# marella/ctransformers

Measured on NVIDIA H100. Metric: decode tokens/s Llama-2-7B Q4_K_M b=1, higher is better.
Workload: dtype int8 (q4_K/q6_K weights x q8_K activations, mma.sync u8 x s8 -> exact int32), fp32 combine in the reference's order

## Files before the change

### ctransformers_b200/csrc/engine.cu

```cuda
#include "engine.cuh"

#include <algorithm>
#include <chrono>
#include <cstdio>
#include <cstring>
#include <stdexcept>

#include "attention.cuh"
#include "grammar.hpp"
#include "grammar_gpu.cuh"
#include "matvec.cuh"
#include "prefill.cuh"
#include "repack.cuh"
#include "sample_gpu.cuh"
#include "score_gpu.cuh"
#include "stream.cuh"
#include "tables.hpp"
#include "tp_nccl.hpp"

namespace ctb {

#define CTB_CUDA(expr)                                                                                         \
  do {                                                                                                         \
    cudaError_t e__ = (expr);                                                                                  \
// ... 328 lines not shown
  xa_ = (float*)alloc(hp_.n_embd * 4); xb_ = (float*)alloc(hp_.n_embd * 4);
  qkv_ = (float*)alloc(qkv * 4);
  attn_ = (float*)alloc(hp_.n_embd * 4); attn_o_ = (float*)alloc(hp_.n_embd * 4);
  ffn_ = (float*)alloc((size_t)nff_ * 4);
  ffn2_ = (float*)alloc((size_t)nff_ * 4);
  d_logits_ = (float*)alloc((size_t)hp_.n_vocab * 4);
  d_embd_ = (float*)alloc(hp_.n_embd * 4);
  {
    const size_t nl = (size_t)hp_.n_seq * hp_.n_vocab, ne = (size_t)hp_.n_seq * hp_.n_embd, bytes = (nl + ne) * 4 + (size_t)hp_.n_seq * 8;
    kept_logits_ = (float*)alloc(bytes);
    kept_embd_ = kept_logits_ + nl;
    kept_pick_ = (int*)(kept_embd_ + ne);
    CTB_CUDA(cudaMemset(kept_logits_, 0, bytes));
  }
  d_sync_ = (unsigned*)alloc(64);
  CTB_CUDA(cudaMemset(d_state_, 0, 64));
  CTB_CUDA(cudaMemset(d_sync_, 0, 64));
  h_logits_ = HostMem((size_t)hp_.n_vocab * 4);
  h_embd_ = HostMem((size_t)hp_.n_embd * 4);
  memset(h_logits_.get(), 0, (size_t)hp_.n_vocab * 4);
  memset(h_embd_.get(), 0, (size_t)hp_.n_embd * 4);
  step_ring_ = StateRing(d_state_, 4, 512);

  if (const char* e = getenv("CTB_NO_PDL")) pdl_ = !(e[0] == '1');
  if (const char* e = getenv("CTB_NO_SPEC")) spec_on_ = !(e[0] == '1');
  if (const char* e = getenv("CTB_STEP_FUSE")) fused_ = !(e[0] == '0');
  if (const char* e = getenv("CTB_NO_PREFILL")) prefill_on_ = !(e[0] == '1');
  if (const char* e = getenv("CTB_PREFILL_MIN")) prefill_min_ = std::max(1, atoi(e));
  h_spec_tok_ = HostMem(16);
  {
// ... 239 lines not shown
    push_matvec(p, MVK_OUT);
    mark_exchange(first_op);

  }
  {
    StepOp op{};
    op.ph.kind = PH_PICK;
    op.ph.pk.logits = d_logits_; op.ph.pk.state = d_state_; op.ph.pk.out_tokens = nullptr; op.ph.pk.n = hp_.n_vocab;
    ops_.push_back(op);
  }
  bool any_stream = false;
  for (const StepOp& op : ops_) any_stream |= op.ph.kind == PH_MATVEC && op.stream;
  std::vector<Phase> phs;
  for (const StepOp& op : ops_) if (op.ph.kind != PH_XCHG && (op.ph.kind != PH_MATVEC || op.stream)) phs.push_back(op.ph);
  const StepLaunch sl = step_launch_plan(phs.data(), (int)phs.size(), sm_count_);
  step_grid_ = sl.grid; step_slots_ = sl.n_slots; step_smem_ = sl.smem; step_q3_ = sl.q3;
  if (const char* e = getenv("CTB_ST_SLOTS")) {
    const int want = atoi(e);
    if (want >= ST_W && want < step_slots_ && want % ST_W == 0) { step_smem_ -= (size_t)(step_slots_ - want) * ST_SLOT; step_slots_ = want; }
  }
  ring_attn_ = st_attn_ring_ok(hp_.n_ctx, step_slots_) && !getenv("CTB_NO_RING_ATTN");
  for (StepOp& op : ops_) if (op.ph.kind == PH_ATTN) op.ph.q6 = ring_attn_ ? 1 : 0;
  if (any_stream && step_slots_ < ST_W) throw std::runtime_error("model rows are too long for the step kernel's shared memory");
  if (any_stream) {
    CTB_CUDA(step_set_smem_limit(step_smem_));
    StepLaunch pl = sl;
    pl.n_slots = step_slots_; pl.smem = step_smem_;
    step_pair_ = step_pair_choose(pl, phs.data(), (int)phs.size());
  } else {
    fused_ = false;
  }
  d_prog_ = (Phase*)alloc((ops_.size() + 1) * sizeof(Phase), 256);
  d_prog_mv_ = (Phase*)alloc((ops_.size() + 1) * sizeof(Phase), 256);
  d_bounds_ = (int*)alloc((ops_.size() + 1) * (size_t)(sm_count_ + 1) * 4, 256);
  d_bounds_mv_ = (int*)alloc((ops_.size() + 1) * (size_t)(sm_count_ + 1) * 4, 256);
}

void Engine::upload_prog(Phase* dst, int* dst_bounds, const std::vector<StepOp>& ops) {
  std::vector<Phase> phs(ops.size());
  for (size_t i = 0; i < ops.size(); i++) phs[i] = ops[i].ph;
  CTB_CUDA(cudaMemcpy(dst, phs.data(), phs.size() * sizeof(Phase), cudaMemcpyHostToDevice));
  std::vector<Phase> run = phs;
  for (size_t i = 0; i < ops.size(); i++) if (ops[i].ph.kind == PH_XCHG || (ops[i].ph.kind == PH_MATVEC && !ops[i].stream)) run[i].kind = -1;
  const std::vector<int> b = step_bounds(run.data(), (int)run.size(), sm_count_);
  CTB_CUDA(cudaMemcpy(dst_bounds, b.data(), b.size() * 4, cudaMemcpyHostToDevice));
}

struct ProfMark {
  Event ev;
  int kind;
};

long Engine::enqueue_ops(const std::vector<StepOp>& ops, const Phase* d_prog, const int* d_bounds, int n, cudaStream_t st, bool fused,
                         std::vector<ProfMark>* marks) {
  long launches = 0;
  auto mark = [&](int kind) {
    if (!marks) return;
    marks->push_back({Event(cudaEventDefault), kind});
    CTB_CUDA(cudaEventRecord(marks->back().ev, st));
  };
  StepLaunch step_shape_;
  step_shape_.grid = step_grid_; step_shape_.n_slots = step_slots_; step_shape_.smem = step_smem_; step_shape_.gen = !attn_fast_hd(hp_.head_dim());
  step_shape_.q3 = step_q3_;
  step_shape_.pair = step_pair_;
  auto capable = [&](const StepOp& op) { return op.ph.kind != PH_XCHG && (op.ph.kind != PH_MATVEC || op.stream); };
  int i = 0;
  while (i < n) {
    const StepOp& op = ops[i];
    if (fused && capable(op)) {
      int j = i;
      while (j < n && capable(ops[j])) j++;
      mark(-1);
      CTB_CUDA(launch_step(step_shape_, st, d_prog + i, d_bounds + (size_t)i * (sm_count_ + 1), j - i, d_sync_, false, nullptr, tp_peer_));
      launches++;
      mark(0);
      i = j;
      continue;
    }
    mark(-1);
    switch (op.ph.kind) {
      case PH_EMBED:
        k_embed<<<1, 256, 0, st>>>(op.ph.em);
        launches++;
        mark(3);
        break;
      case PH_ATTN:
        CTB_CUDA(launch_kernel(attn_kernel(hp_.head_dim()), dim3(nh_, 1, attn_groups(hp_.head_dim())), dim3(ATTN_THREADS), attn_smem_bytes(hp_.n_ctx, hp_.head_dim()), st, pdl_, op.ph.at));
        launches++;
        mark(1);
        break;
      case PH_XCHG:
        tp_all_reduce(op.ph.em.out, op.ph.em.K, st);
        mark(3);
        break;
      case PH_PICK:
        k_argmax<<<1, ARGMAX_THREADS, 0, st>>>(d_logits_, hp_.n_vocab, d_state_ + 4);
        k_advance<<<1, 1, 0, st>>>(d_state_, d_tokens_out_.as<int>());
        launches += 2;
        mark(3);
        break;
      default:
        if (op.stream) {
          CTB_CUDA(launch_step(step_shape_, st, d_prog + i, d_bounds + (size_t)i * (sm_count_ + 1), 1, d_sync_));
        } else {
          const MVLaunch L = matvec_launch_shape(op.ph.mv, sm_count_);
          CTB_CUDA(launch_matvec_kernel(L, st, op.ph.mv, pdl_));
        }
        launches++;
        mark(0);
    }
    i++;
  }
  CTB_CUDA(cudaGetLastError());
  return launches;
}

int Engine::profile_step(int token, int n_past, double ms_by_kind[4], int count_by_kind[4]) {
  DeviceGuard dev_guard(device_);
// ... 45 lines not shown
  return (double)ms / reps;
}

long Engine::trace_step(int token, int n_past, unsigned long long* out, long cap_words) {
  DeviceGuard dev_guard(device_);
  if (tp_.world > 1) throw std::runtime_error("not available in tensor-parallel mode (every rank must run the same launches)");
  drop_lookahead();
  const int n = n_body_ + 1;
  for (int i = 0; i < n; i++)
    if (ops_[i].ph.kind == PH_MATVEC && !ops_[i].stream) return 0;
  const long need = 2L * n + 8L * n * step_grid_;
  if (need > cap_words) return -need;
  const DevMem buf((size_t)n * step_grid_ * 64);
  CTB_CUDA(cudaMemset(buf.get(), 0, (size_t)n * step_grid_ * 64));
  StepLaunch L;
  L.grid = step_grid_; L.n_slots = step_slots_; L.smem = step_smem_; L.gen = !attn_fast_hd(hp_.head_dim()); L.q3 = step_q3_; L.pair = step_pair_;
  for (int rep = 0; rep < 3; rep++) {
    put_step(token, n_past, n_past + 1);
    CTB_CUDA(launch_step(L, stream_, d_prog_, d_bounds_, n, d_sync_, false, buf.as<unsigned long long>()));
    CTB_CUDA(cudaStreamSynchronize(stream_));
  }
  for (int i = 0; i < n; i++) { out[2 * i] = (unsigned long long)ops_[i].ph.kind; out[2 * i + 1] = (unsigned long long)ops_[i].mvk; }
  CTB_CUDA(cudaMemcpy(out + 2 * n, buf.get(), (size_t)n * step_grid_ * 64, cudaMemcpyDeviceToHost));
  return n;
}

void Engine::build_graphs() {
  tokens_out_cap_ = std::max(hp_.n_ctx, 4096);
  d_tokens_out_ = DevMem((size_t)tokens_out_cap_ * 4);
  h_tokens_out_ = HostMem((size_t)tokens_out_cap_ * 4);
  const Stream cap(cudaStreamNonBlocking);
  ops_.back().ph.pk.out_tokens = d_tokens_out_.as<int>();
  upload_prog(d_prog_, d_bounds_, ops_);
  long launches = 0;
// ... 770 lines not shown
```

### ctransformers_b200/csrc/engine.cuh

```cuda
#pragma once
#include <cmath>
#include <memory>
#include <string>
#include <vector>

#include "cuda_owned.cuh"
#include "device_types.cuh"
#include "gguf.hpp"

namespace ctb {

struct TPShard {
  int rank = 0, world = 1;
  int head0 = 0, head1 = 0, kv0 = 0, kv1 = 0, ff0 = 0, ff1 = 0;
  void* comm = nullptr;
};
TPShard tp_shard(int n_embd, int n_head, int n_head_kv, int n_ff, int rank, int world);

struct HParams {
  bool falcon = false;
  int n_vocab = 0, n_ctx_train = 0, n_embd = 0, n_ff = 0, n_head = 0, n_head_kv = 0, n_layer = 0, n_rot = 0;
  float eps = 1e-5f, rope_base = 10000.f, rope_scale = 1.f;
  int n_ctx = 512;
  int n_seq = 1;
// ... 128 lines not shown
  int kv_high_ = 0;
  HostMem h_spec_tok_;
  HostMem h_dbg_;
  void after_eval(int next_pos);
  int sm_count_ = 132;

  void init(const GGUFFile& g);
  DevMat upload_matrix(const GGUFTensor& t, struct Uploader& up, int want_K, int want_M, int row0 = 0, int row1 = -1, int k0 = 0, int k1 = -1);
  const float* upload_vector(const GGUFFile& g, const std::string& name, bool required, int want_n);
  std::vector<StepOp> ops_;
  int n_body_ = 0;
  Phase* d_prog_ = nullptr;
  Phase* d_prog_mv_ = nullptr;
  int *d_bounds_ = nullptr, *d_bounds_mv_ = nullptr;
  unsigned* d_sync_ = nullptr;
  int step_grid_ = 0, step_slots_ = 0;
  size_t step_smem_ = 0;
  bool fused_ = true;
  bool step_q3_ = false;
  bool step_pair_ = false;
  bool ring_attn_ = false;
  void build_ops();
  void push_matvec(struct MVParams& p, int kind);
  void upload_prog(Phase* dst, int* dst_bounds, const std::vector<StepOp>& ops);
  long enqueue_ops(const std::vector<StepOp>& ops, const Phase* d_prog, const int* d_bounds, int n, cudaStream_t st, bool fused,
                   std::vector<ProfMark>* marks = nullptr);
  void build_graphs();
  bool eager_ = false;
  bool host_fresh_ = true;
  void host_views();
  DevMem d_sample_;
  HostMem h_sample_;
  void sample_enqueue(const SampleRow* rows, int R, bool picks);
  bool pieces_ready_ = false;
  DevMem d_pieces_, d_gm_, d_gm_rows_;
// ... 45 lines not shown
```

### ctransformers_b200/csrc/matvec.cuh

```cuda
#pragma once
#include "device_types.cuh"
#include "attention.cuh"

namespace ctb {

#ifndef CTB_THREADS
#define CTB_THREADS 512
#endif
constexpr int MV_THREADS = CTB_THREADS;
constexpr int MV_WARPS = MV_THREADS / 32;
constexpr int MV_ROWS = 4;
constexpr int MV_MAX_SEG = 3;

enum : int { NORM_NONE = 0, NORM_RMS = 1, NORM_LAYER = 2 };
enum : int { EPI_STORE = 0, EPI_ADD = 1, EPI_GELU = 2, EPI_ADD2 = 3, EPI_SILU = 4 };

#ifndef ST_WATCHDOG_NS
#define ST_WATCHDOG_NS 4000000000ull
#endif
#ifndef XC_WATCHDOG_NS
#define XC_WATCHDOG_NS 30000000000ull
#endif
enum WaitCode : int {
  W_GRID_BARRIER = 1, W_FOLD_FLAG, W_FREE_WEIGHT_SLOT, W_WEIGHT_ITEM, W_FREE_K_SLOT, W_FREE_V_SLOT, W_K_ITEM, W_V_ITEM, W_XCHG,
  W_PF_GRID_BARRIER, W_PF_FREE_SLOT, W_PF_WEIGHT_ITEM, W_PAIR, W_CODES
};
constexpr const char* WAIT_TEXT[] = {"?", "grid barrier (aux = phase)", "fold hand-off flag (aux = chunk)", "producer: free weight slot (aux = item)",
                                     "consumer: weight item (aux = item)", "producer: free K slot (attention)", "producer: free V slot (attention)",
                                     "consumer: K item (attention)", "consumer: V item (attention)", "tensor-parallel exchange: a peer's element (aux = exchange number)",
// ... 16 lines not shown
}

struct MVSeg {
  DevMat w;
  float* out;
  const float* res;
  const float* res2;
  int epi;
};

struct MVParams {
  const float* x;
  const float* x2;
  int x_mode;
  int x_parts, x_stride;
  float* sum_out;
  const float* norm_w;
  const float* norm_b;
  float* norm_out;
  float eps;
  int norm_mode;
  int K;
  int act;
  int nseg;
  MVSeg seg[MV_MAX_SEG];
  const uint16_t* silu_tab;
  const uint16_t* gelu_tab;
};

struct ActView {
// ... 209 lines not shown
    for (int l = 0; l < 32; l++)
#pragma unroll
      for (int i = 0; i < 16; i++) {
        float t = __shfl_sync(0xffffffffu, v[i], l);
        if (kind == NORM_TERM_DEV) t = __fsub_rn(t, mean);
        if (base + l * 16 + i < K) seq += kind == NORM_TERM_X ? (double)t : (double)__fmul_rn(t, t);
      }
  }
  return seq;
}

template <int NT, int BAR, bool XC, bool PAIR = false>
__device__ __forceinline__ float norm_stat(double s, double a, double g, bool a_is_s, int kind, float mean, const MVParams& xs, double* red,
                                           unsigned epoch, PairX* px = nullptr) {
  const int K = xs.K;
  if constexpr (PAIR) pair_sum2_max_f64<NT, BAR>(s, a, g, a_is_s, *px);
  else if (a_is_s) a = s = block_sum_f64<NT, BAR>(s, red);
  else block_sum2_max_f64<NT, BAR>(s, a, g, red);
  if (!isfinite(s) || (!a_is_s && __dmul_ru(a, g) < 0x1p52)) return (float)(s / (double)K);
  const double e = __dmul_ru(a, (double)K * 0x1.0000001p-52);
  const float lo = (float)(__dsub_rd(s, e) / (double)K), hi = (float)(__dadd_ru(s, e) / (double)K);
  if (lo == hi) return lo;
  const double seq = threadIdx.x < 32 ? seq_sum_warp0<XC>(xs.x, xs.x2, xs.x_mode, xs.x_parts, xs.x_stride, K, kind, mean, epoch) : 0.0;
  bar_sync<BAR, NT>();
  if (threadIdx.x == 0) red[0] = seq;
  bar_sync<BAR, NT>();
  return (float)(red[0] / (double)K);
}

__device__ __forceinline__ void norm_apply16(float (&v)[16], const float (&w)[16], const float (&bb)[16], int norm_mode, float mean, float scale, bool has_w,
                                             bool has_b) {
// ... 178 lines not shown
      }
    } else if (act == ACT_F16) {
      uint16_t* h = (uint16_t*)smem;
#pragma unroll
      for (int e = 0; e < 16; e++) if (e < valid) h[base + e] = f2h(v[e]);
    } else {
      float* f = (float*)smem;
#pragma unroll
      for (int e = 0; e < 16; e++) if (e < valid) f[base + e] = v[e];
    }
  }
  bar_sync<BAR, NT>();
}

template <int NT, int BAR>
__device__ __forceinline__ void stage_q8k_pair(const MVParams& xs, const NormPre& np, uint8_t* smem, double* red, PairX& px, bool write_norm) {
  const int K = xs.K, nb = K >> 8, norm_mode = xs.norm_mode, t = threadIdx.x, lane = t & 31;
  const int lo = pair_block0(nb, (int)px.rank) * 256, hi = pair_block0(nb, (int)px.rank + 1) * 256;
  const int base[2] = {lo + t * 16, lo + (t + NT) * 16};
  float v[2][16];
  load16x(xs, base[0], hi - base[0], v[0]);
  load16x(xs, base[1], hi - base[1], v[1]);
  float mean = 0.f, scale = 1.f;
  if (norm_mode == NORM_RMS) {
    double ss = 0.0;
#pragma unroll
    for (int h = 0; h < 2; h++)
#pragma unroll
      for (int e = 0; e < 16; e++) ss += (double)__fmul_rn(v[h][e], v[h][e]);
    const float m = norm_stat<NT, BAR, false, true>(ss, ss, 0.0, true, NORM_TERM_SQ, 0.f, xs, red, 0, &px);
    scale = __fdiv_rn(1.0f, __fsqrt_rn(__fadd_rn(m, xs.eps)));
  } else if (norm_mode == NORM_LAYER) {
    double s1 = 0.0, a1 = 0.0;
    unsigned emin = 255;
#pragma unroll
    for (int h = 0; h < 2; h++)
#pragma unroll
      for (int e = 0; e < 16; e++) {
        s1 += (double)v[h][e];
        a1 += (double)fabsf(v[h][e]);
// ... 233 lines not shown
```

### ctransformers_b200/csrc/stream.cuh

```cuda
#pragma once
#include <stdexcept>
#include <string>
#include "matvec.cuh"

namespace ctb {

#ifndef CTB_ST_WARPS
#define CTB_ST_WARPS 10
#endif
constexpr int ST_W = CTB_ST_WARPS;
constexpr int ST_NT = ST_W * 32;
constexpr int ST_THREADS = ST_NT + 32;
constexpr int ST_SLOT = 9216;
#ifndef CTB_ST_DEPTH
#define CTB_ST_DEPTH 2
#endif
constexpr int ST_MAX_DEPTH = CTB_ST_DEPTH;
constexpr int ST_MAX_SLOTS = ST_W * ST_MAX_DEPTH;
constexpr int ST_MAXT = 16;
constexpr int ST_ROWS = 16;
constexpr int ST_BAR = 1;
constexpr int ST_STATE = 6;

#ifndef CTB_CHUNK_Q3
// ... 365 lines not shown
    const uint32_t w0 = __vsub4((a0 & 0x0f0f0f0fu) | ((a2 & 0x03030303u) << 4), 0x20202020u);
    const uint32_t w1 = __vsub4((a1 & 0x0f0f0f0fu) | (((a2 >> 2) & 0x03030303u) << 4), 0x20202020u);
    const uint32_t w2 = __vsub4(((a0 >> 4) & 0x0f0f0f0fu) | (((a2 >> 4) & 0x03030303u) << 4), 0x20202020u);
    const uint32_t w3 = __vsub4(((a1 >> 4) & 0x0f0f0f0fu) | (((a2 >> 6) & 0x03030303u) << 4), 0x20202020u);
    const uint32_t sel = par ? 0x7531u : 0x6420u;
    const uint32_t S0 = __byte_perm(w0, w1, sel), S1 = __byte_perm(w2, w3, sel);
#pragma unroll
    for (int c = 0; c < 2; c++) {
      const int i = rr * 2 + c;
      r.p[i] = (float)scale_fold8(D[0][i], D[1][i], D[2][i], D[3][i], D[4][i], D[5][i], D[6][i], D[7][i], S0, S1);
    }
    r.dd[rr] = __fmul_rn(yd, h2f(rr ? d1 : d0));
  }
}

template <int TYPE, bool XC>
__device__ __forceinline__ void run_item(const uint8_t* slot, uint64_t* empty_bar, int nblk, int b0, int kc, bool last, const StAct& a, int lane,
                                         volatile float* mail, volatile int* flag, const MVSeg& sg, const MVParams& p, int row0) {
  constexpr int KB = StTraits<TYPE>::KB, BB = StTraits<TYPE>::BB, NM = StTraits<TYPE>::NM;
  Terms tr[KB];
  if (nblk == KB) {
#pragma unroll
    for (int i = 0; i < KB; i++) block_terms<TYPE>(slot + i * BB, b0 + i, a, lane, tr[i]);
  } else {
#pragma unroll
    for (int i = 0; i < KB; i++) {
      if (i < nblk) block_terms<TYPE>(slot + i * BB, b0 + i, a, lane, tr[i]);
      else { Terms z{}; tr[i] = z; }
    }
  }
  __syncwarp();
  if (lane == 0) mbar_arrive(empty_bar);

// ... 35 lines not shown
    u0 = __fadd_rn(u0, __shfl_xor_sync(0xffffffffu, u0, 2));
    u1 = __fadd_rn(u1, __shfl_xor_sync(0xffffffffu, u1, 2));
    u0 = __fadd_rn(u0, __shfl_xor_sync(0xffffffffu, u0, 1));
    u1 = __fadd_rn(u1, __shfl_xor_sync(0xffffffffu, u1, 1));
    float v = __fadd_rn(u0, u1);
    if (TYPE == GT_Q4_K) {
      float m = accm[rr];
      m = __fadd_rn(m, __shfl_xor_sync(0xffffffffu, m, 2));
      m = __fadd_rn(m, __shfl_xor_sync(0xffffffffu, m, 1));
      v = __fadd_rn(v, m);
    } else if (TYPE == GT_Q5_K) {
      v = __fadd_rn(v, __shfl_sync(0xffffffffu, accm[0], (lane & ~3) + rr));
    }
    out[rr] = v;
  }
  if (t < 2) {
    const int row = row0 + g + 8 * t;
    if (row < sg.w.M) {
      if (XC && a.xc) {
        const float v = epilogue(sg.epi, t ? out[1] : out[0], sg.res + row, sg.res2 + row, p);
        const XchgParams& xc = *a.xc;
        const size_t at = ((size_t)(a.epoch & 1u) * xc.world + xc.rank) * xc.n + row;
        for (int r = 0; r < xc.world; r++)
          asm volatile("st.volatile.global.v2.u32 [%0], {%1, %2};" ::"l"(xc.ll[r] + at), "r"(__float_as_uint(v)), "r"(a.epoch) : "memory");
      } else {
        store_epilogue(sg, p, row, t ? out[1] : out[0]);
      }
    }
  }
}

struct TileSpace {
  int tiles[MV_MAX_SEG], cost[MV_MAX_SEG], nseg, ntiles;
  long total;
  template <bool Q3 = true>
  __host__ __device__ __forceinline__ void init(const MVParams& p) {
    nseg = p.nseg; ntiles = 0; total = 0;
#pragma unroll
    for (int s = 0; s < MV_MAX_SEG; s++) {
      tiles[s] = s < p.nseg ? (p.seg[s].w.M + ST_ROWS - 1) / ST_ROWS : 0;
      cost[s] = s < p.nseg ? st_tile_cost<Q3>(p.seg[s].w.type) : 1;
      ntiles += tiles[s]; total += (long)tiles[s] * cost[s];
    }
// ... 34 lines not shown
  int q6;
  MVParams mv;
  AttnParams at;
  EmbedParams em;
  PickParams pk;
  XchgParams xc;
};

struct StepArgs {
  const Phase* prog;
  int n_phases;
  int n_slots;
  unsigned* sync;
  const int* bounds;
  unsigned long long* trace;
};

__device__ __forceinline__ unsigned ld_relaxed_u32(const unsigned* p) {
  unsigned v;
  asm volatile("ld.relaxed.gpu.global.u32 %0, [%1];" : "=r"(v) : "l"(p) : "memory");
  return v;
}
__device__ __forceinline__ unsigned ld_acquire_u32(const unsigned* p) {
  unsigned v;
  asm volatile("ld.acquire.gpu.global.u32 %0, [%1];" : "=r"(v) : "l"(p) : "memory");
  return v;
}

struct TileInfo { int seg, til, nch, type; };
template <bool Q3>
// ... 121 lines not shown
  const int n_cg = GEN ? attn_groups(ph.at.hd) : ph.at.hd / ATTN_CH, n_tasks = ph.at.n_head * n_cg, G = (int)gridDim.x;
  if (ph.q6) {
    const AttnRing ag = attn_ring_geom<GEN>(ph.at);
    for (int task = blockIdx.x; task < n_tasks; task += G) {
      if (task != (int)blockIdx.x) bar_sync<ST_BAR, ST_NT>();
      if (ag.T > 0) st_attn_task<GEN>(ph.at, act_smem, ring, full_bar, empty_bar, (uint32_t)(n_slots / ST_W), seq, ag, task / n_cg, task % n_cg, pick_v, red);
      seq += (uint32_t)(ag.n_k + attn_ring_nv<GEN>(ag, ph.at.hd, task % n_cg));
    }
  } else {
    for (int task = blockIdx.x; task < n_tasks; task += G) {
      if (task != (int)blockIdx.x) bar_sync<ST_BAR, ST_NT>();
      attn_body<ST_NT, ST_BAR, false, GEN>(ph.at, act_smem, task / n_cg, 0, task % n_cg, ph.at.state);
    }
  }
}
template <bool Q3, bool PAIR>
static __device__ __noinline__ uint32_t st_attn_phase_gen(const Phase& ph, uint8_t* act_smem, uint8_t* ring, uint64_t* full_bar, uint64_t* empty_bar, int n_slots,
                                                   uint32_t seq, float* pick_v, double* red) {
  st_attn_phase<true>(ph, act_smem, ring, full_bar, empty_bar, n_slots, seq, pick_v, red);
  return seq;
}

template <bool XC, bool GEN, bool Q3>
__device__ __forceinline__ void st_producer(const StepArgs& args, uint8_t* ring, uint64_t* full_bar, uint64_t* empty_bar) {
  const int lane = threadIdx.x & 31;
  const uint32_t S = (uint32_t)(args.n_slots / ST_W);
  const uint64_t weight_pol = l2_policy_evict_first();
  uint32_t seq = 0;
  for (int ip = 0; ip < args.n_phases; ip++) {
    const Phase* ph = args.prog + ip;
    if (ph->kind == PH_ATTN) {
// ... 23 lines not shown
            const RingPos rp = st_ring(n, S);
            const StItem it = st_item<Q3>(p, ti.seg, ti.type, ti.til, kc, nb);
            mbar_wait(&empty_bar[rp.slot], rp.parity ^ 1u, W_FREE_WEIGHT_SLOT, (int)n);
            mbar_expect_tx(&full_bar[rp.slot], it.bytes);
            bulk_g2s_hint(ring + (size_t)rp.slot * ST_SLOT, it.src, it.bytes, &full_bar[rp.slot], weight_pol);
          }
          __syncwarp();
        }
        __syncwarp();
        seq += (uint32_t)__popc(mask);
      }
    }
  }
}

template <bool XC, bool Q3, bool PAIR>
__device__ __forceinline__ void st_matvec_phase(const Phase& ph, const NormPre& np, uint8_t* ring, uint8_t* act_smem, double* red, uint64_t* full_bar, uint64_t* empty_bar,
                                                float (*mailbox)[ST_STATE * 32], int* flags, uint32_t S, uint32_t& seq, const int* tb, unsigned long long* tr,
                                                unsigned xc_base, PairX& px) {
  const MVParams& p = ph.mv;
  const int warp = threadIdx.x >> 5, lane = threadIdx.x & 31;
  const unsigned epoch = XC ? xc_base + (unsigned)ph.xc.index + 1u : 0u;
  if constexpr (PAIR) stage_q8k_pair<ST_NT, ST_BAR>(p, np, act_smem, red, px, blockIdx.x < 2);
  else stage_activation<ST_NT, ST_BAR, XC>(p, np, ACT_Q8_K, act_smem, red, blockIdx.x == 0, epoch);
  StAct a = st_act_extras<ST_NT, ST_BAR>(act_smem, p.K, ph.q6 != 0);
  a.xc = XC && ph.xc.role == 2 ? &ph.xc : nullptr;
  a.epoch = epoch;
  if (tr && threadIdx.x == 0) tr[1] = globaltimer_ns();
  bool first_item = tr != nullptr && threadIdx.x == 0;
  TileSpace ts;
  ts.init<Q3>(p);
  const int nb = p.K >> 8;
  const int T0 = tb[0], T1 = tb[1];
#pragma unroll 1
  for (int w0 = T0; w0 < T1; w0 += ST_MAXT) {
    if (w0 != T0) {
      bar_sync<ST_BAR, ST_NT>();
      if (threadIdx.x < ST_MAXT) flags[threadIdx.x] = 0;
      bar_sync<ST_BAR, ST_NT>();
// ... 11 lines not shown
        for (int q = 0; q < r; q++) mr &= mr - 1;
        const int j = __ffs(mr) - 1;
        const int seg = __shfl_sync(0xffffffffu, ti.seg, j), til = __shfl_sync(0xffffffffu, ti.til, j), type = __shfl_sync(0xffffffffu, ti.type, j);
        const int nch = __shfl_sync(0xffffffffu, ti.nch, j);
        const uint32_t n = seq + (uint32_t)r;
        const RingPos rp = st_ring(n, S);
        const int kb = st_chunk_blocks<Q3>(type);
        const int b0 = kc * kb, nblk = min(kb, nb - b0);
        const MVSeg& sg = p.seg[seg];
        const uint8_t* sp = ring + (size_t)rp.slot * ST_SLOT;
        mbar_wait(&full_bar[rp.slot], rp.parity, W_WEIGHT_ITEM, (int)n);
        if (first_item) { tr[2] = globaltimer_ns(); first_item = false; }
        volatile float* mail = mailbox[j];
        volatile int* flag = flags + j;
        const bool last = kc == nch - 1;
        if (type == GT_Q4_K) run_item<GT_Q4_K, XC>(sp, &empty_bar[rp.slot], nblk, b0, kc, last, a, lane, mail, flag, sg, p, til * ST_ROWS);
        else if (type == GT_Q6_K) run_item<GT_Q6_K, XC>(sp, &empty_bar[rp.slot], nblk, b0, kc, last, a, lane, mail, flag, sg, p, til * ST_ROWS);
        else if (Q3 && type == GT_Q3_K) run_item<GT_Q3_K, XC>(sp, &empty_bar[rp.slot], nblk, b0, kc, last, a, lane, mail, flag, sg, p, til * ST_ROWS);
        else run_item<GT_Q5_K, XC>(sp, &empty_bar[rp.slot], nblk, b0, kc, last, a, lane, mail, flag, sg, p, til * ST_ROWS);
      }
      seq += (uint32_t)cnt;
    }
  }
}

__device__ __forceinline__ void st_pick_phase(const PickParams& pk, float* bv, int* bi) {
  float best;
  int idx;
  block_argmax<ST_NT, ST_BAR, true>(pk.logits, pk.n, bv, bi, best, idx);
  if (threadIdx.x == 0) {
    pk.state[4] = idx;
    advance_state(pk.state, pk.out_tokens, idx);
  }
}

__device__ __forceinline__ void grid_rearm(unsigned* sync, bool set_xc = false, unsigned xc = 0) {
  if (threadIdx.x == 0) {
    __threadfence();
    if (atomicAdd(sync + 1, 1u) == gridDim.x - 1) {
      sync[0] = 0u;
      sync[1] = 0u;
      if (set_xc) sync[2] = xc;
      __threadfence();
    }
  }
}

template <bool XC, bool GEN, bool Q3, bool PAIR = false>
static __global__ void __launch_bounds__(ST_THREADS, 1) k_step(const __grid_constant__ StepArgs args) {
  extern __shared__ __align__(16) uint8_t smem[];
  __shared__ __align__(8) uint64_t full_bar[ST_MAX_SLOTS];
  __shared__ __align__(8) uint64_t empty_bar[ST_MAX_SLOTS];
  __shared__ double red[3 * ST_W];
  __shared__ __align__(16) float mailbox[ST_MAXT][ST_STATE * 32];
  __shared__ int flags[ST_MAXT];
  __shared__ float pick_v[ST_W];
  __shared__ int pick_i[ST_W];
  __shared__ __align__(16) Phase ph_s[2];
  __shared__ int tb_s[2][2];
  __shared__ __align__(8) uint64_t pair_bar[PAIR ? 2 : 1];
  __shared__ double pair_red[PAIR ? 2 * 2 * 3 * ST_W : 1];
  const int warp = threadIdx.x >> 5;
  uint8_t* ring = smem;
// ... 7 lines not shown
      asm volatile("fence.mbarrier_init.release.cluster;" ::: "memory");
    }
    px.rank = cluster_ctarank();
    asm volatile("barrier.cluster.arrive.release.aligned;\n barrier.cluster.wait.acquire.aligned;" ::: "memory");
  }
  pdl_trigger();
  pdl_wait();
  if (warp == ST_W) {
    st_producer<XC, GEN, Q3>(args, ring, full_bar, empty_bar);
    return;
  }
  const unsigned G = gridDim.x;
  uint32_t seq = 0;
  const unsigned xc_base = XC ? ld_relaxed_u32(args.sync + 2) : 0u;
  unsigned xc_done = 0;
  auto fetch_phase = [&](int ip) {
    if (ip >= args.n_phases) return;
    const uint4* src = (const uint4*)(args.prog + ip);
    const uint32_t dst = st_smem(&ph_s[ip & 1]);
    const int i = (int)threadIdx.x - 32;
    if (i >= 0 && i < (int)(sizeof(Phase) / 16)) asm volatile("cp.async.ca.shared.global [%0], [%1], 16;" ::"r"(dst + i * 16), "l"(src + i) : "memory");
    if (i >= 64 && i < 66)
      asm volatile("cp.async.ca.shared.global [%0], [%1], 4;" ::"r"(st_smem(&tb_s[ip & 1][i - 64])), "l"(args.bounds + (size_t)ip * (gridDim.x + 1) + blockIdx.x + (i - 64)) : "memory");
    asm volatile("cp.async.commit_group;" ::: "memory");
  };
  fetch_phase(0);
#pragma unroll 1
  for (int ip = 0; ip < args.n_phases; ip++) {
    bar_sync<ST_BAR, ST_NT>();
    unsigned long long* const tr = args.trace ? args.trace + ((size_t)ip * G + blockIdx.x) * 8 : nullptr;
    if (tr && threadIdx.x == 0) tr[4] = globaltimer_ns();
    if (threadIdx.x == 0 && ip > 0) {
      const unsigned target = (unsigned)ip * G;
      asm volatile("red.release.gpu.global.add.u32 [%0], 1;" ::"l"(args.sync) : "memory");
      if (tr) tr[5] = globaltimer_ns();
      bounded_wait([&] { return ld_relaxed_u32(args.sync) >= target; }, W_GRID_BARRIER, ip);
      if (tr) { tr[6] = globaltimer_ns(); tr[7] = tr[6]; }
    } else {
      asm volatile("cp.async.wait_all;" ::: "memory");
      if (threadIdx.x >= 32 && threadIdx.x < 32 + ST_MAXT) flags[threadIdx.x - 32] = 0;
    }
    bar_sync<ST_BAR, ST_NT>();
    const Phase& ph = ph_s[ip & 1];
    fetch_phase(ip + 1);
    NormPre np;
    if (ph.kind == PH_MATVEC) preload_norm(np, ph.mv, PAIR ? pair_block0(ph.mv.K >> 8, (int)px.rank) * 256 : 0);
    if (tr && threadIdx.x == 0) tr[0] = globaltimer_ns();
    if (XC && ph.kind == PH_MATVEC && ph.xc.role == 1) xc_done++;
    if (ph.kind == PH_MATVEC) {
      st_matvec_phase<XC, Q3, PAIR>(ph, np, ring, act_smem, red, full_bar, empty_bar, mailbox, flags, (uint32_t)(args.n_slots / ST_W), seq, &tb_s[ip & 1][0], tr,
                                    xc_base, px);
    } else if (ph.kind == PH_ATTN) {
      if (GEN) seq = st_attn_phase_gen<Q3, PAIR>(ph, act_smem, ring, full_bar, empty_bar, args.n_slots, seq, pick_v, red);
      else st_attn_phase<false>(ph, act_smem, ring, full_bar, empty_bar, args.n_slots, seq, pick_v, red);
    } else if (ph.kind == PH_EMBED) {
      if (blockIdx.x == 0) embed_row<Q3>(ph.em, ph.em.tokens[0], ph.em.out, threadIdx.x, ST_NT);
    } else if (ph.kind == PH_PICK) {
      if (blockIdx.x == 0) st_pick_phase(ph.pk, pick_v, pick_i);
    }
    if (tr) {
      bar_sync<ST_BAR, ST_NT>();
      if (threadIdx.x == 0) tr[3] = globaltimer_ns();
    }
  }
  bar_sync<ST_BAR, ST_NT>();
  grid_rearm(args.sync, XC, xc_base + xc_done);
}

struct StepLaunch { int grid; int n_slots; size_t smem; bool gen = false, q3 = false, pair = false;  };

inline StepLaunch step_launch_shape(const Phase* phases, int n, int n_sm, size_t max_dyn_smem, size_t extra_act = 0) {
  size_t act = extra_act;
  for (int i = 0; i < n; i++) {
    if (phases[i].kind == PH_MATVEC) act = std::max(act, st_act_bytes(phases[i].mv.K, phases[i].q6 != 0));
    if (phases[i].kind == PH_ATTN) act = std::max(act, attn_smem_bytes(phases[i].at.n_ctx, phases[i].at.hd));
  }
  bool gen = false, q3 = false;
  for (int i = 0; i < n; i++) {
    gen |= phases[i].kind == PH_ATTN && !attn_fast_hd(phases[i].at.hd);
    if (phases[i].kind == PH_MATVEC)
      for (int s = 0; s < phases[i].mv.nseg; s++) q3 |= phases[i].mv.seg[s].w.type == GT_Q3_K;
    q3 |= phases[i].kind == PH_EMBED && phases[i].em.type == GT_Q3_K;
  }
  act = (act + 127) & ~(size_t)127;
  StepLaunch L;
  L.grid = n_sm;
  L.gen = gen;
  L.q3 = q3;
  if (act + (size_t)ST_W * ST_SLOT > max_dyn_smem) { L.n_slots = 0; L.smem = 0; return L; }
  L.n_slots = ST_W * (int)std::min<size_t>(ST_MAX_DEPTH, (max_dyn_smem - act) / ((size_t)ST_W * ST_SLOT));
  L.smem = (size_t)L.n_slots * ST_SLOT + act;
  return L;
}

inline std::vector<int> step_bounds(const Phase* phs, int n, int grid) {
  std::vector<int> b((size_t)n * (grid + 1), 0);
  for (int i = 0; i < n; i++) {
    if (phs[i].kind != PH_MATVEC) continue;
    TileSpace ts;
    ts.init(phs[i].mv);
    for (int c = 0; c <= grid; c++) b[(size_t)i * (grid + 1) + c] = ts.boundary(c, grid);
  }
  return b;
// ... 19 lines not shown
static inline cudaError_t st_set_debug_words(int* dev_ptr) { return cudaMemcpyToSymbol(g_st_dbg, &dev_ptr, sizeof(int*)); }
static inline cudaError_t step_set_smem_limit(size_t bytes) {
  void (*const kernels[])(StepArgs) = {k_step<false, false, false>, k_step<false, true, false>, k_step<true, false, false>,
                                        k_step<false, false, true>, k_step<false, true, true>, k_step<true, false, true>};
  for (auto k : kernels) {
    const cudaError_t e = cudaFuncSetAttribute(k, cudaFuncAttributeMaxDynamicSharedMemorySize, (int)bytes);
    if (e != cudaSuccess) return e;
  }
  return cudaSuccess;
}

inline bool step_paired(const StepLaunch& L, bool xchg) { return L.pair && !L.q3 && !xchg; }
using StepKernel = void (*)(StepArgs);
inline StepKernel step_kernel(const StepLaunch& L, bool xchg) {
  if (xchg) return L.q3 ? k_step<true, false, true> : k_step<true, false, false>;
  if (step_paired(L, xchg)) return L.gen ? k_step<false, true, false, true> : k_step<false, false, false, true>;
  return L.q3 ? (L.gen ? k_step<false, true, true> : k_step<false, false, true>) : (L.gen ? k_step<false, true, false> : k_step<false, false, false>);
}

inline bool step_pair_fits(const Phase* phases, int n) {
  for (int i = 0; i < n; i++)
    if (phases[i].kind == PH_MATVEC && pair_block0(phases[i].mv.K >> 8, 1) * 16 > 2 * ST_NT) return false;
  return true;
}

inline bool step_pair_wanted() {
  const char* e = getenv("CTB_ST_CLUSTER");
  return !(e && e[0] == '0');
}

inline StepLaunch step_launch_plan(const Phase* phases, int n, int n_sm, size_t extra_act = 0) {
  StepLaunch L = step_launch_shape(phases, n, n_sm, max_dyn_smem(k_step<true, false, false>), extra_act);
  if (!L.q3 && step_pair_wanted())
    L = step_launch_shape(phases, n, n_sm, std::min(max_dyn_smem(k_step<false, false, false, true>), max_dyn_smem(k_step<false, true, false, true>)), extra_act);
  return L;
}

inline bool step_pair_choose(StepLaunch& L, const Phase* phases, int n) {
  L.pair = false;
  if (!step_pair_wanted() || L.q3 || L.grid % 2 || !step_pair_fits(phases, n)) return false;
  StepLaunch P = L;
  P.pair = true;
  const StepKernel k = step_kernel(P, false);
  auto check = [](cudaError_t e) {
    if (e != cudaSuccess) throw std::runtime_error(std::string("pairing the step kernel: ") + cudaGetErrorString(e));
  };
  check(cudaFuncSetAttribute(k, cudaFuncAttributeMaxDynamicSharedMemorySize, (int)L.smem));
  cudaLaunchConfig_t cfg{};
  cfg.gridDim = dim3(L.grid); cfg.blockDim = dim3(ST_THREADS); cfg.dynamicSmemBytes = L.smem;
  cudaLaunchAttribute at[1];
  at[0].id = cudaLaunchAttributeClusterDimension;
  at[0].val.clusterDim.x = 2; at[0].val.clusterDim.y = 1; at[0].val.clusterDim.z = 1;
  cfg.attrs = at; cfg.numAttrs = 1;
  int clusters = 0;
  check(cudaOccupancyMaxActiveClusters(&clusters, k, &cfg));
  L.pair = clusters >= L.grid / 2;
  return L.pair;
}

static inline cudaError_t launch_step(const StepLaunch& L, cudaStream_t st, const Phase* d_prog, const int* d_bounds, int n_phases, unsigned* d_sync, bool pdl = false,
                                      unsigned long long* trace = nullptr, bool xchg = false) {
  StepArgs a;
  a.prog = d_prog; a.bounds = d_bounds; a.n_phases = n_phases; a.n_slots = L.n_slots; a.sync = d_sync; a.trace = trace;
  return launch_kernel_cluster(step_kernel(L, xchg), dim3(L.grid), dim3(ST_THREADS), L.smem, st, pdl, step_paired(L, xchg) ? 2u : 1u, a);
}

}
```

Before: 376.6.

## Fuse RMS-norm sum-of-squares into producing matvec epilogue via per-block partials

When a matvec's output feeds directly into an RMS-normed matvec, the producer now accumulates the sum of squares of its outputs in its epilogue. Each block writes its partial to a global array at the grid barrier. The consumer then reads all per-block partials instead of re-reducing the full activation vector before quantizing it. This removes a block-wide reduction and a pass over the input from the consumer's staging step. In exchange it adds an atomic per warp, an extra kernel template variant, and a changed summation order for the norm statistic.

```diff
diff --git a/ctransformers_b200/csrc/engine.cu b/ctransformers_b200/csrc/engine.cu
--- a/ctransformers_b200/csrc/engine.cu
+++ b/ctransformers_b200/csrc/engine.cu
@@ -366,6 +366,7 @@
     CTB_CUDA(cudaMemset(kept_logits_, 0, bytes));
   }
   d_sync_ = (unsigned*)alloc(64);
+  d_ss_part_ = (double*)alloc((size_t)sm_count_ * sizeof(double));
   CTB_CUDA(cudaMemset(d_state_, 0, 64));
   CTB_CUDA(cudaMemset(d_sync_, 0, 64));
   h_logits_ = HostMem((size_t)hp_.n_vocab * 4);
@@ -635,7 +636,7 @@
   std::vector<Phase> phs;
   for (const StepOp& op : ops_) if (op.ph.kind != PH_XCHG && (op.ph.kind != PH_MATVEC || op.stream)) phs.push_back(op.ph);
   const StepLaunch sl = step_launch_plan(phs.data(), (int)phs.size(), sm_count_);
-  step_grid_ = sl.grid; step_slots_ = sl.n_slots; step_smem_ = sl.smem; step_q3_ = sl.q3;
+  step_grid_ = sl.grid; step_slots_ = sl.n_slots; step_smem_ = sl.smem; step_q3_ = sl.q3; step_stat_ = sl.stat;
   if (const char* e = getenv("CTB_ST_SLOTS")) {
     const int want = atoi(e);
     if (want >= ST_W && want < step_slots_ && want % ST_W == 0) { step_smem_ -= (size_t)(step_slots_ - want) * ST_SLOT; step_slots_ = want; }
@@ -660,9 +661,18 @@
 void Engine::upload_prog(Phase* dst, int* dst_bounds, const std::vector<StepOp>& ops) {
   std::vector<Phase> phs(ops.size());
   for (size_t i = 0; i < ops.size(); i++) phs[i] = ops[i].ph;
-  CTB_CUDA(cudaMemcpy(dst, phs.data(), phs.size() * sizeof(Phase), cudaMemcpyHostToDevice));
   std::vector<Phase> run = phs;
   for (size_t i = 0; i < ops.size(); i++) if (ops[i].ph.kind == PH_XCHG || (ops[i].ph.kind == PH_MATVEC && !ops[i].stream)) run[i].kind = -1;
+  if (sm_count_ <= 32 * ST_STAT_LANE)
+    for (size_t i = 1; i < ops.size(); i++) {
+      const Phase &w = run[i - 1], &r = run[i];
+      if (r.kind == PH_MATVEC && w.kind == PH_MATVEC && r.mv.norm_mode == NORM_RMS && r.mv.x_mode == 0 && w.mv.nseg == 1 && w.mv.seg[0].out == r.mv.x &&
+          w.mv.seg[0].w.M == r.mv.K && !(w.mv.stat & ST_STAT_CONSUME)) {
+        phs[i - 1].mv.stat |= ST_STAT_PRODUCE; phs[i].mv.stat |= ST_STAT_CONSUME;
+        run[i - 1].mv.stat |= ST_STAT_PRODUCE; run[i].mv.stat |= ST_STAT_CONSUME;
+      }
+    }
+  CTB_CUDA(cudaMemcpy(dst, phs.data(), phs.size() * sizeof(Phase), cudaMemcpyHostToDevice));
   const std::vector<int> b = step_bounds(run.data(), (int)run.size(), sm_count_);
   CTB_CUDA(cudaMemcpy(dst_bounds, b.data(), b.size() * 4, cudaMemcpyHostToDevice));
 }
@@ -683,7 +693,7 @@
   StepLaunch step_shape_;
   step_shape_.grid = step_grid_; step_shape_.n_slots = step_slots_; step_shape_.smem = step_smem_; step_shape_.gen = !attn_fast_hd(hp_.head_dim());
   step_shape_.q3 = step_q3_;
-  step_shape_.pair = step_pair_;
+  step_shape_.pair = step_pair_; step_shape_.stat = step_stat_;
   auto capable = [&](const StepOp& op) { return op.ph.kind != PH_XCHG && (op.ph.kind != PH_MATVEC || op.stream); };
   int i = 0;
   while (i < n) {
@@ -692,7 +702,7 @@
       int j = i;
       while (j < n && capable(ops[j])) j++;
       mark(-1);
-      CTB_CUDA(launch_step(step_shape_, st, d_prog + i, d_bounds + (size_t)i * (sm_count_ + 1), j - i, d_sync_, false, nullptr, tp_peer_));
+      CTB_CUDA(launch_step(step_shape_, st, d_prog + i, d_bounds + (size_t)i * (sm_count_ + 1), j - i, d_sync_, false, nullptr, tp_peer_, d_ss_part_));
       launches++;
       mark(0);
       i = j;
@@ -722,7 +732,7 @@
         break;
       default:
         if (op.stream) {
-          CTB_CUDA(launch_step(step_shape_, st, d_prog + i, d_bounds + (size_t)i * (sm_count_ + 1), 1, d_sync_));
+          CTB_CUDA(launch_step(step_shape_, st, d_prog + i, d_bounds + (size_t)i * (sm_count_ + 1), 1, d_sync_, false, nullptr, false, d_ss_part_));
         } else {
           const MVLaunch L = matvec_launch_shape(op.ph.mv, sm_count_);
           CTB_CUDA(launch_matvec_kernel(L, st, op.ph.mv, pdl_));
@@ -798,10 +808,10 @@
   const DevMem buf((size_t)n * step_grid_ * 64);
   CTB_CUDA(cudaMemset(buf.get(), 0, (size_t)n * step_grid_ * 64));
   StepLaunch L;
-  L.grid = step_grid_; L.n_slots = step_slots_; L.smem = step_smem_; L.gen = !attn_fast_hd(hp_.head_dim()); L.q3 = step_q3_; L.pair = step_pair_;
+  L.grid = step_grid_; L.n_slots = step_slots_; L.smem = step_smem_; L.gen = !attn_fast_hd(hp_.head_dim()); L.q3 = step_q3_; L.pair = step_pair_; L.stat = step_stat_;
   for (int rep = 0; rep < 3; rep++) {
     put_step(token, n_past, n_past + 1);
-    CTB_CUDA(launch_step(L, stream_, d_prog_, d_bounds_, n, d_sync_, false, buf.as<unsigned long long>()));
+    CTB_CUDA(launch_step(L, stream_, d_prog_, d_bounds_, n, d_sync_, false, buf.as<unsigned long long>(), false, d_ss_part_));
     CTB_CUDA(cudaStreamSynchronize(stream_));
   }
   for (int i = 0; i < n; i++) { out[2 * i] = (unsigned long long)ops_[i].ph.kind; out[2 * i + 1] = (unsigned long long)ops_[i].mvk; }
diff --git a/ctransformers_b200/csrc/engine.cuh b/ctransformers_b200/csrc/engine.cuh
--- a/ctransformers_b200/csrc/engine.cuh
+++ b/ctransformers_b200/csrc/engine.cuh
@@ -166,11 +166,13 @@
   Phase* d_prog_mv_ = nullptr;
   int *d_bounds_ = nullptr, *d_bounds_mv_ = nullptr;
   unsigned* d_sync_ = nullptr;
+  double* d_ss_part_ = nullptr;
   int step_grid_ = 0, step_slots_ = 0;
   size_t step_smem_ = 0;
   bool fused_ = true;
   bool step_q3_ = false;
   bool step_pair_ = false;
+  bool step_stat_ = false;
   bool ring_attn_ = false;
   void build_ops();
   void push_matvec(struct MVParams& p, int kind);
diff --git a/ctransformers_b200/csrc/matvec.cuh b/ctransformers_b200/csrc/matvec.cuh
--- a/ctransformers_b200/csrc/matvec.cuh
+++ b/ctransformers_b200/csrc/matvec.cuh
@@ -13,6 +13,8 @@
 constexpr int MV_MAX_SEG = 3;
 
 enum : int { NORM_NONE = 0, NORM_RMS = 1, NORM_LAYER = 2 };
+enum : int { ST_STAT_PRODUCE = 1, ST_STAT_CONSUME = 2 };
+constexpr int ST_STAT_LANE = 5;
 enum : int { EPI_STORE = 0, EPI_ADD = 1, EPI_GELU = 2, EPI_ADD2 = 3, EPI_SILU = 4 };
 
 #ifndef ST_WATCHDOG_NS
@@ -59,6 +61,7 @@
   const float* x2;
   int x_mode;
   int x_parts, x_stride;
+  int stat;
   float* sum_out;
   const float* norm_w;
   const float* norm_b;
@@ -298,7 +301,7 @@
 __device__ __forceinline__ float norm_stat(double s, double a, double g, bool a_is_s, int kind, float mean, const MVParams& xs, double* red,
                                            unsigned epoch, PairX* px = nullptr) {
   const int K = xs.K;
-  if constexpr (PAIR) pair_sum2_max_f64<NT, BAR>(s, a, g, a_is_s, *px);
+  if constexpr (PAIR) { if (px) pair_sum2_max_f64<NT, BAR>(s, a, g, a_is_s, *px); }
   else if (a_is_s) a = s = block_sum_f64<NT, BAR>(s, red);
   else block_sum2_max_f64<NT, BAR>(s, a, g, red);
   if (!isfinite(s) || (!a_is_s && __dmul_ru(a, g) < 0x1p52)) return (float)(s / (double)K);
@@ -507,16 +510,29 @@
 }
 
 template <int NT, int BAR>
-__device__ __forceinline__ void stage_q8k_pair(const MVParams& xs, const NormPre& np, uint8_t* smem, double* red, PairX& px, bool write_norm) {
+__device__ __forceinline__ void stage_q8k_pair(const MVParams& xs, const NormPre& np, uint8_t* smem, double* red, PairX& px, bool write_norm,
+                                               const double* ss_part = nullptr, int n_part = 0) {
   const int K = xs.K, nb = K >> 8, norm_mode = xs.norm_mode, t = threadIdx.x, lane = t & 31;
   const int lo = pair_block0(nb, (int)px.rank) * 256, hi = pair_block0(nb, (int)px.rank + 1) * 256;
   const int base[2] = {lo + t * 16, lo + (t + NT) * 16};
+  double ss = 0.0;
+  if (ss_part) {
+    double q[ST_STAT_LANE];
+#pragma unroll
+    for (int i = 0; i < ST_STAT_LANE; i++) q[i] = lane + 32 * i < n_part ? __ldcg(ss_part + lane + 32 * i) : 0.0;
+#pragma unroll
+    for (int i = 0; i < ST_STAT_LANE; i++) ss += q[i];
+  }
   float v[2][16];
   load16x(xs, base[0], hi - base[0], v[0]);
   load16x(xs, base[1], hi - base[1], v[1]);
   float mean = 0.f, scale = 1.f;
-  if (norm_mode == NORM_RMS) {
-    double ss = 0.0;
+  if (norm_mode == NORM_RMS && ss_part) {
+#pragma unroll
+    for (int o = 16; o > 0; o >>= 1) ss += __shfl_xor_sync(0xffffffffu, ss, o);
+    const float m = norm_stat<NT, BAR, false, true>(ss, ss, 0.0, true, NORM_TERM_SQ, 0.f, xs, red, 0, nullptr);
+    scale = __fdiv_rn(1.0f, __fsqrt_rn(__fadd_rn(m, xs.eps)));
+  } else if (norm_mode == NORM_RMS) {
 #pragma unroll
     for (int h = 0; h < 2; h++)
 #pragma unroll
diff --git a/ctransformers_b200/csrc/stream.cuh b/ctransformers_b200/csrc/stream.cuh
--- a/ctransformers_b200/csrc/stream.cuh
+++ b/ctransformers_b200/csrc/stream.cuh
@@ -403,9 +403,9 @@
   }
 }
 
-template <int TYPE, bool XC>
+template <int TYPE, bool XC, bool STAT>
 __device__ __forceinline__ void run_item(const uint8_t* slot, uint64_t* empty_bar, int nblk, int b0, int kc, bool last, const StAct& a, int lane,
-                                         volatile float* mail, volatile int* flag, const MVSeg& sg, const MVParams& p, int row0) {
+                                         volatile float* mail, volatile int* flag, const MVSeg& sg, const MVParams& p, int row0, double* ss_acc) {
   constexpr int KB = StTraits<TYPE>::KB, BB = StTraits<TYPE>::BB, NM = StTraits<TYPE>::NM;
   Terms tr[KB];
   if (nblk == KB) {
@@ -471,6 +471,7 @@
     }
     out[rr] = v;
   }
+  double sq = 0.0;
   if (t < 2) {
     const int row = row0 + g + 8 * t;
     if (row < sg.w.M) {
@@ -480,10 +481,19 @@
         const size_t at = ((size_t)(a.epoch & 1u) * xc.world + xc.rank) * xc.n + row;
         for (int r = 0; r < xc.world; r++)
           asm volatile("st.volatile.global.v2.u32 [%0], {%1, %2};" ::"l"(xc.ll[r] + at), "r"(__float_as_uint(v)), "r"(a.epoch) : "memory");
+      } else if (STAT && ss_acc) {
+        const float v = epilogue(sg.epi, t ? out[1] : out[0], sg.res + row, sg.res2 + row, p);
+        sg.out[row] = v;
+        sq = (double)__fmul_rn(v, v);
       } else {
         store_epilogue(sg, p, row, t ? out[1] : out[0]);
       }
     }
+  }
+  if (STAT && ss_acc) {
+#pragma unroll
+    for (int o = 16; o > 0; o >>= 1) sq += __shfl_xor_sync(0xffffffffu, sq, o);
+    if (lane == 0) atomicAdd(ss_acc, sq);
   }
 }
 
@@ -548,6 +558,7 @@
   unsigned* sync;
   const int* bounds;
   unsigned long long* trace;
+  double* ss_part;
 };
 
 __device__ __forceinline__ unsigned ld_relaxed_u32(const unsigned* p) {
@@ -699,7 +710,7 @@
     }
   }
 }
-template <bool Q3, bool PAIR>
+template <bool Q3, bool PAIR, bool STAT>
 static __device__ __noinline__ uint32_t st_attn_phase_gen(const Phase& ph, uint8_t* act_smem, uint8_t* ring, uint64_t* full_bar, uint64_t* empty_bar, int n_slots,
                                                    uint32_t seq, float* pick_v, double* red) {
   st_attn_phase<true>(ph, act_smem, ring, full_bar, empty_bar, n_slots, seq, pick_v, red);
@@ -753,15 +764,18 @@
   }
 }
 
-template <bool XC, bool Q3, bool PAIR>
+template <bool XC, bool Q3, bool PAIR, bool STAT>
 __device__ __forceinline__ void st_matvec_phase(const Phase& ph, const NormPre& np, uint8_t* ring, uint8_t* act_smem, double* red, uint64_t* full_bar, uint64_t* empty_bar,
                                                 float (*mailbox)[ST_STATE * 32], int* flags, uint32_t S, uint32_t& seq, const int* tb, unsigned long long* tr,
-                                                unsigned xc_base, PairX& px) {
+                                                unsigned xc_base, PairX& px, const double* ss_part) {
   const MVParams& p = ph.mv;
   const int warp = threadIdx.x >> 5, lane = threadIdx.x & 31;
   const unsigned epoch = XC ? xc_base + (unsigned)ph.xc.index + 1u : 0u;
-  if constexpr (PAIR) stage_q8k_pair<ST_NT, ST_BAR>(p, np, act_smem, red, px, blockIdx.x < 2);
+  if constexpr (STAT) stage_q8k_pair<ST_NT, ST_BAR>(p, np, act_smem, red, px, blockIdx.x < 2, ss_part, (int)gridDim.x);
+  else if constexpr (PAIR) stage_q8k_pair<ST_NT, ST_BAR>(p, np, act_smem, red, px, blockIdx.x < 2);
   else stage_activation<ST_NT, ST_BAR, XC>(p, np, ACT_Q8_K, act_smem, red, blockIdx.x == 0, epoch);
+  double* const ss_acc = STAT && (p.stat & ST_STAT_PRODUCE) ? red + 3 * ST_W - 1 : nullptr;
+  if (ss_acc && threadIdx.x == 0) *ss_acc = 0.0;
   StAct a = st_act_extras<ST_NT, ST_BAR>(act_smem, p.K, ph.q6 != 0);
   a.xc = XC && ph.xc.role == 2 ? &ph.xc : nullptr;
   a.epoch = epoch;
@@ -803,10 +817,10 @@
         volatile float* mail = mailbox[j];
         volatile int* flag = flags + j;
         const bool last = kc == nch - 1;
-        if (type == GT_Q4_K) run_item<GT_Q4_K, XC>(sp, &empty_bar[rp.slot], nblk, b0, kc, last, a, lane, mail, flag, sg, p, til * ST_ROWS);
-        else if (type == GT_Q6_K) run_item<GT_Q6_K, XC>(sp, &empty_bar[rp.slot], nblk, b0, kc, last, a, lane, mail, flag, sg, p, til * ST_ROWS);
-        else if (Q3 && type == GT_Q3_K) run_item<GT_Q3_K, XC>(sp, &empty_bar[rp.slot], nblk, b0, kc, last, a, lane, mail, flag, sg, p, til * ST_ROWS);
-        else run_item<GT_Q5_K, XC>(sp, &empty_bar[rp.slot], nblk, b0, kc, last, a, lane, mail, flag, sg, p, til * ST_ROWS);
+        if (type == GT_Q4_K) run_item<GT_Q4_K, XC, STAT>(sp, &empty_bar[rp.slot], nblk, b0, kc, last, a, lane, mail, flag, sg, p, til * ST_ROWS, ss_acc);
+        else if (type == GT_Q6_K) run_item<GT_Q6_K, XC, STAT>(sp, &empty_bar[rp.slot], nblk, b0, kc, last, a, lane, mail, flag, sg, p, til * ST_ROWS, ss_acc);
+        else if (Q3 && type == GT_Q3_K) run_item<GT_Q3_K, XC, STAT>(sp, &empty_bar[rp.slot], nblk, b0, kc, last, a, lane, mail, flag, sg, p, til * ST_ROWS, ss_acc);
+        else run_item<GT_Q5_K, XC, STAT>(sp, &empty_bar[rp.slot], nblk, b0, kc, last, a, lane, mail, flag, sg, p, til * ST_ROWS, ss_acc);
       }
       seq += (uint32_t)cnt;
     }
@@ -835,7 +849,7 @@
   }
 }
 
-template <bool XC, bool GEN, bool Q3, bool PAIR = false>
+template <bool XC, bool GEN, bool Q3, bool PAIR = false, bool STAT = false>
 static __global__ void __launch_bounds__(ST_THREADS, 1) k_step(const __grid_constant__ StepArgs args) {
   extern __shared__ __align__(16) uint8_t smem[];
   __shared__ __align__(8) uint64_t full_bar[ST_MAX_SLOTS];
@@ -873,6 +887,7 @@
   uint32_t seq = 0;
   const unsigned xc_base = XC ? ld_relaxed_u32(args.sync + 2) : 0u;
   unsigned xc_done = 0;
+  bool prev_prod = false;
   auto fetch_phase = [&](int ip) {
     if (ip >= args.n_phases) return;
     const uint4* src = (const uint4*)(args.prog + ip);
@@ -890,6 +905,7 @@
     unsigned long long* const tr = args.trace ? args.trace + ((size_t)ip * G + blockIdx.x) * 8 : nullptr;
     if (tr && threadIdx.x == 0) tr[4] = globaltimer_ns();
     if (threadIdx.x == 0 && ip > 0) {
+      if (STAT && prev_prod) args.ss_part[blockIdx.x] = red[3 * ST_W - 1];
       const unsigned target = (unsigned)ip * G;
       asm volatile("red.release.gpu.global.add.u32 [%0], 1;" ::"l"(args.sync) : "memory");
       if (tr) tr[5] = globaltimer_ns();
@@ -907,10 +923,10 @@
     if (tr && threadIdx.x == 0) tr[0] = globaltimer_ns();
     if (XC && ph.kind == PH_MATVEC && ph.xc.role == 1) xc_done++;
     if (ph.kind == PH_MATVEC) {
-      st_matvec_phase<XC, Q3, PAIR>(ph, np, ring, act_smem, red, full_bar, empty_bar, mailbox, flags, (uint32_t)(args.n_slots / ST_W), seq, &tb_s[ip & 1][0], tr,
-                                    xc_base, px);
+      st_matvec_phase<XC, Q3, PAIR, STAT>(ph, np, ring, act_smem, red, full_bar, empty_bar, mailbox, flags, (uint32_t)(args.n_slots / ST_W), seq, &tb_s[ip & 1][0], tr,
+                                    xc_base, px, STAT && prev_prod && (ph.mv.stat & ST_STAT_CONSUME) ? args.ss_part : nullptr);
     } else if (ph.kind == PH_ATTN) {
-      if (GEN) seq = st_attn_phase_gen<Q3, PAIR>(ph, act_smem, ring, full_bar, empty_bar, args.n_slots, seq, pick_v, red);
+      if (GEN) seq = st_attn_phase_gen<Q3, PAIR, STAT>(ph, act_smem, ring, full_bar, empty_bar, args.n_slots, seq, pick_v, red);
       else st_attn_phase<false>(ph, act_smem, ring, full_bar, empty_bar, args.n_slots, seq, pick_v, red);
     } else if (ph.kind == PH_EMBED) {
       if (blockIdx.x == 0) embed_row<Q3>(ph.em, ph.em.tokens[0], ph.em.out, threadIdx.x, ST_NT);
@@ -921,12 +937,13 @@
       bar_sync<ST_BAR, ST_NT>();
       if (threadIdx.x == 0) tr[3] = globaltimer_ns();
     }
+    if constexpr (STAT) prev_prod = ph.kind == PH_MATVEC && (ph.mv.stat & ST_STAT_PRODUCE);
   }
   bar_sync<ST_BAR, ST_NT>();
   grid_rearm(args.sync, XC, xc_base + xc_done);
 }
 
-struct StepLaunch { int grid; int n_slots; size_t smem; bool gen = false, q3 = false, pair = false;  };
+struct StepLaunch { int grid; int n_slots; size_t smem; bool gen = false, q3 = false, pair = false, stat = false;  };
 
 inline StepLaunch step_launch_shape(const Phase* phases, int n, int n_sm, size_t max_dyn_smem, size_t extra_act = 0) {
   size_t act = extra_act;
@@ -934,9 +951,10 @@
     if (phases[i].kind == PH_MATVEC) act = std::max(act, st_act_bytes(phases[i].mv.K, phases[i].q6 != 0));
     if (phases[i].kind == PH_ATTN) act = std::max(act, attn_smem_bytes(phases[i].at.n_ctx, phases[i].at.hd));
   }
-  bool gen = false, q3 = false;
+  bool gen = false, q3 = false, stat = false;
   for (int i = 0; i < n; i++) {
     gen |= phases[i].kind == PH_ATTN && !attn_fast_hd(phases[i].at.hd);
+    stat |= phases[i].kind == PH_MATVEC && phases[i].mv.norm_mode == NORM_RMS;
     if (phases[i].kind == PH_MATVEC)
       for (int s = 0; s < phases[i].mv.nseg; s++) q3 |= phases[i].mv.seg[s].w.type == GT_Q3_K;
     q3 |= phases[i].kind == PH_EMBED && phases[i].em.type == GT_Q3_K;
@@ -946,6 +964,7 @@
   L.grid = n_sm;
   L.gen = gen;
   L.q3 = q3;
+  L.stat = stat;
   if (act + (size_t)ST_W * ST_SLOT > max_dyn_smem) { L.n_slots = 0; L.smem = 0; return L; }
   L.n_slots = ST_W * (int)std::min<size_t>(ST_MAX_DEPTH, (max_dyn_smem - act) / ((size_t)ST_W * ST_SLOT));
   L.smem = (size_t)L.n_slots * ST_SLOT + act;
@@ -995,6 +1014,7 @@
 using StepKernel = void (*)(StepArgs);
 inline StepKernel step_kernel(const StepLaunch& L, bool xchg) {
   if (xchg) return L.q3 ? k_step<true, false, true> : k_step<true, false, false>;
+  if (step_paired(L, xchg) && L.stat) return L.gen ? k_step<false, true, false, true, true> : k_step<false, false, false, true, true>;
   if (step_paired(L, xchg)) return L.gen ? k_step<false, true, false, true> : k_step<false, false, false, true>;
   return L.q3 ? (L.gen ? k_step<false, true, true> : k_step<false, false, true>) : (L.gen ? k_step<false, true, false> : k_step<false, false, false>);
 }
@@ -1013,7 +1033,8 @@
 inline StepLaunch step_launch_plan(const Phase* phases, int n, int n_sm, size_t extra_act = 0) {
   StepLaunch L = step_launch_shape(phases, n, n_sm, max_dyn_smem(k_step<true, false, false>), extra_act);
   if (!L.q3 && step_pair_wanted())
-    L = step_launch_shape(phases, n, n_sm, std::min(max_dyn_smem(k_step<false, false, false, true>), max_dyn_smem(k_step<false, true, false, true>)), extra_act);
+    L = step_launch_shape(phases, n, n_sm, std::min({max_dyn_smem(k_step<false, false, false, true>), max_dyn_smem(k_step<false, true, false, true>),
+                                                     max_dyn_smem(k_step<false, false, false, true, true>), max_dyn_smem(k_step<false, true, false, true, true>)}), extra_act);
   return L;
 }
 
@@ -1040,9 +1061,9 @@
 }
 
 static inline cudaError_t launch_step(const StepLaunch& L, cudaStream_t st, const Phase* d_prog, const int* d_bounds, int n_phases, unsigned* d_sync, bool pdl = false,
-                                      unsigned long long* trace = nullptr, bool xchg = false) {
+                                      unsigned long long* trace = nullptr, bool xchg = false, double* ss_part = nullptr) {
   StepArgs a;
-  a.prog = d_prog; a.bounds = d_bounds; a.n_phases = n_phases; a.n_slots = L.n_slots; a.sync = d_sync; a.trace = trace;
+  a.prog = d_prog; a.bounds = d_bounds; a.n_phases = n_phases; a.n_slots = L.n_slots; a.sync = d_sync; a.trace = trace; a.ss_part = ss_part;
   return launch_kernel_cluster(step_kernel(L, xchg), dim3(L.grid), dim3(ST_THREADS), L.smem, st, pdl, step_paired(L, xchg) ? 2u : 1u, a);
 }
 
```

New measurement: 380.6 (median of 6 runs). 1.01x the previous value.
